# FYTalon/pienerf

Measured on AMD Instinct MI355X. Metric: sim+render steps/s @800x800 chair, higher is better.
Workload: dtype f32 render / f64 sim

## Files before the change

### include/pienerf_hip.h

```cpp
#ifndef PIENERF_HIP_H
#define PIENERF_HIP_H
#include <stdint.h>
#ifdef __cplusplus
extern "C" {
#endif

#define PN_OK 0
#define PN_ERR_ARG 1
#define PN_ERR_HIP 2
#define PN_ERR_CAPACITY 3

const char* pn_version(void);

int pn_stream_create_cu_mask(uint32_t total_cu, uint32_t first_cu, uint32_t n_cu, int invert, void** stream_out);
int pn_stream_destroy(void* stream);
int pn_march_set_tail_rounds(int rounds);
int pn_march_set_skip_dda(int on);
int pn_device_cu_count(void);
const char* pn_last_error(void);


int pn_sph_from_ray(const float* rays_o, const float* rays_d, float radius, uint32_t N, float* coords, void* stream);
int pn_near_far_from_aabb(const float* rays_o, const float* rays_d, const float* aabb, uint32_t N, float min_near, float* nears, float* fars,
                          void* stream);
// ... 148 lines not shown


typedef struct pn_copier pn_copier;
int pn_copier_create(pn_copier** out);
void pn_copier_destroy(pn_copier* c);
int pn_copier_submit(pn_copier* c, void* dst_host, const void* src_dev, uint64_t bytes, void* after_event, uint64_t* ticket);
int pn_copier_wait(pn_copier* c, uint64_t ticket);


int pn_mark_untrained_grid(const float* poses, uint32_t B, float fx, float fy, float cx, float cy, uint32_t cascade, uint32_t H, float bound,
                           float* density_grid, int* n_unseen, void* stream);
int pn_density_cells_full(uint32_t cascade, uint32_t H, float bound, const float* noise, float* xyzs, void* stream);
int pn_density_cells_partial(uint32_t cas, uint32_t H, float bound, uint32_t N, const int* rand_coords, const float* rand_pick, const float* noise,
                             const float* density_grid_cas, float* tmp_grid_cas, int* scratch, int* indices, float* xyzs, void* stream);
uint64_t pn_density_partial_scratch_ints(uint32_t H);
int pn_density_scatter(uint32_t n, const int* indices, const float* sigmas, float* tmp_grid_cas, void* stream);
int pn_density_grid_update(uint32_t n, float* density_grid, const float* tmp_grid, float decay, float density_thresh, uint8_t* bitfield,
                           double* partial, float* mean_thresh, void* stream);

int pn_frame_march_counters(pn_frame* f, int enable, uint64_t* counters_host, void* stream);
int pn_frame_fused_clocks(pn_frame* f, uint64_t* clocks_host, int* first_trip_out, int reset, void* stream);
int pn_frame_trip_records(pn_frame* f, int* records_host, int* tail_counts_host, int max_trips, void* stream);
int pn_frame_trip_times(pn_frame* f, float* march_ms_host, float* network_ms_host, int max_trips, int* n_trips_out, void* stream);


int pn_sim_update_F(int n_IP, const int* topo, const double* dof, const double* Nx, const double* dNx, const double* ddNx, float* pos, float* F,
                    float* dF, void* stream);

int pn_sim_calc_elastic(int n_IP, const int* topo, const double* dNx, const double* dof, double* RF, double* VF, double* FF, int mcadams_sweeps,
                        void* stream);

int pn_sim_collect_rhs(int n_k, double dx, const int* csr_bg, const int* csr_cnt, const int* csr_buf, const double* mu, const double* lam,
                       const double* dNx, const double* RF, const double* VF, double* rhs, void* stream);

int pn_sim_matvec3(int n, const double* A, const double* X, double* Y, void* stream);

int pn_sim_stepforward(int n_k, int n_IP, int iters, double dt, double dx, const int* topo, const int* csr_bg, const int* csr_cnt,
                       const int* csr_buf, const double* mu, const double* lam, const double* dNx, const double* dNx_csr, const int* csr_pos,
                       const double* Ainv,
                       const double* Mmat, const double* dof_rest, const double* rhs_rest, const double* rhs_gravity, const double* dof_f,
                       double* dof, double* dof_vel, double* work, int prepared, int mcadams_sweeps, void* stream);
uint64_t pn_sim_work_doubles(int n_k, int n_IP);
int pn_sim_cells_chunk_ips(void);
uint64_t pn_sim_cells_work_doubles(int n_k, int n_chunks);
int pn_sim_cells_prepare(int n_k, int n_chunks, double* work, void* stream);
int pn_sim_stepforward_cells(int n_k, int n_chunks, int iters, double dt, double dx, const int* chunk_tab, const double* dNx_cell, const double* mu_cell,
// ... 49 lines not shown
```

### pienerf_amd/_lib.py

```python
import ctypes as C
import os

_HERE = os.path.dirname(os.path.abspath(__file__))
LIB_PATH = os.environ.get("PN_LIB_PATH") or os.path.join(_HERE, "lib", "libpienerf_hip.so")

P = C.c_void_p
u32, i32, f32, f64, u64 = C.c_uint32, C.c_int, C.c_float, C.c_double, C.c_uint64


class RenderOpts(C.Structure):
    _fields_ = [("max_iter_num", i32), ("hash_grid_size", f32), ("num_seek_IP", i32), ("IP_dx", f32), ("cut", i32), ("cut_bounds", f32 * 6),
                ("bound", f32), ("min_near", f32), ("dt_gamma", f32), ("max_steps", u32), ("T_thresh", f32), ("cascade", u32), ("grid_size", u32),
                ("density_scale", f32), ("bg_color", f32), ("fp16", i32), ("reuse_tables", i32), ("ray_batch", i32), ("throughput", i32), ("throughput_trips", i32), ("ray_tile_w", i32),
                ("fused_from", i32), ("fused_whole", i32), ("fused_fold", i32), ("fused_grid", i32)]


SIGNATURES = {
    "pn_version": (C.c_char_p, []),
    "pn_last_error": (C.c_char_p, []),
    "pn_stream_create_cu_mask": (i32, [u32, u32, u32, i32, C.POINTER(C.c_void_p)]),
    "pn_stream_destroy": (i32, [P]),
    "pn_device_cu_count": (i32, []),
    "pn_march_set_tail_rounds": (i32, [i32]),
    "pn_march_set_skip_dda": (i32, [i32]),
# ... 44 lines not shown
    "pn_nerf_color_half": (i32, [P, P, P, P, u32, P, P]),
    "pn_render_hier": (i32, [P, P, P, u32, C.POINTER(f32), f32, i32, i32, f32, f32, P, P, P, P, i32, P]),
    "pn_hier_max_samples": (i32, []),
    "pn_frame_create": (i32, [C.POINTER(P), u32, u32, u32]),
    "pn_frame_destroy": (None, [P]),
    "pn_render_deformed": (i32, [P, P, C.POINTER(RenderOpts), P, P, u32, P, P, P, P, i32, P, P, P, P, P, P, P]),
    "pn_render_deformed_async": (i32, [P, P, C.POINTER(RenderOpts), P, P, u32, P, P, P, P, i32, P, P, P, P, P, i32, P]),
    "pn_render_status": (i32, [P, P, i32, P]),
    "pn_frame_reset_unfinished": (i32, [P, P]),
    "pn_render_continue": (i32, [P, P, C.POINTER(RenderOpts), P, P, u32, P, P, P, P, P, P, i32, i32, P]),
    "pn_render_static": (i32, [P, P, C.POINTER(RenderOpts), P, P, u32, P, P, P, P, P, P, P, i32, P]),
    "pn_mark_untrained_grid": (i32, [P, u32, f32, f32, f32, f32, u32, u32, f32, P, P, P]),
    "pn_density_cells_full": (i32, [u32, u32, f32, P, P, P]),
    "pn_density_cells_partial": (i32, [u32, u32, f32, u32, P, P, P, P, P, P, P, P, P]),
    "pn_density_partial_scratch_ints": (u64, [u32]),
    "pn_density_scatter": (i32, [u32, P, P, P, P]),
    "pn_density_grid_update": (i32, [u32, P, P, f32, f32, P, P, P, P]),
    "pn_frame_march_counters": (i32, [P, i32, P, P]),
    "pn_frame_trip_times": (i32, [P, P, P, i32, P, P]),
    "pn_frame_fused_clocks": (i32, [P, P, P, i32, P]),
    "pn_net_form": (i32, [P]),
    "pn_net_form_epoch": (i32, [P]),
    "pn_frame_trip_records": (i32, [P, P, P, i32, P]),
    "pn_sim_update_F": (i32, [i32, P, P, P, P, P, P, P, P, P]),
    "pn_sim_calc_elastic": (i32, [i32, P, P, P, P, P, P, i32, P]),
    "pn_sim_collect_rhs": (i32, [i32, f64, P, P, P, P, P, P, P, P, P, P]),
    "pn_sim_matvec3": (i32, [i32, P, P, P, P]),
    "pn_sim_stepforward": (i32, [i32, i32, i32, f64, f64, P, P, P, P, P, P, P, P, P, P, P, P, P, P, P, P, P, P, i32, i32, P]),
    "pn_sim_prepare": (i32, [i32, i32, P, P, P, P]),
    "pn_sim_cells_chunk_ips": (i32, []),
    "pn_sim_cells_work_doubles": (u64, [i32, i32]),
    "pn_sim_cells_prepare": (i32, [i32, i32, P, P]),
    "pn_sim_stepforward_cells": (i32, [i32, i32, i32, f64, f64, P, P, P, P, P, P, P, P, P, P, P, P, P, P, P, i32, P]),
    "pn_sim_work_doubles": (u64, [i32, i32]),
    "pn_sim_coop_bytes": (u64, [i32, i32, i32]),
    "pn_sim_coop_prepare": (i32, [i32, i32, i32, P, P, P, C.POINTER(i32), P]),
    "pn_sim_coop_status": (i32, [P, C.POINTER(i32)]),
    "pn_sim_coop_clocks": (i32, [P, C.POINTER(u64)]),
    "pn_sim_stepforward_coop": (i32, [i32, i32, i32, f64, f64, P, P, P, P, P, P, P, P, P, P, P, P, P, P, P, P, i32, C.POINTER(i32), P]),
    "pn_sim_update_force": (i32, [i32, i32, P, f64, P, P, P, P, P]),
    "pn_sim_drag_bytes": (u64, []),
    "pn_sim_drag_work_doubles": (u64, []),
    "pn_sim_drag_force": (i32, [i32, i32, P, P, f64, P, P, P, P, P]),
    "pn_sim_drag_set": (i32, [P, i32, i32, i32, f64, P, P]),
    "pn_sim_drag_unproject": (i32, [P, i32, i32, f64, f64, P, P, P, i32, P, P, P]),
    "pn_mc_work_bytes": (u64, [i32, i32, i32]),
# ... 49 lines not shown
```

### pienerf_amd/csrc/pn_render_ops.hip

```cpp
#include <float.h>

#include "pn_render_records.h"
#include "pn_cell_hash.h"
#include "pn_side_tables.h"
#include "pn_march_kernels.h"
#include "pn_composite.h"
#include "pn_compact.h"
#include "pn_frame_kernels.h"

thread_local char pn_err_buf[512] = {0};

extern "C" int pn_pnts_in_grids(int n_vtx, int n_grid, const float* pnts, const float* bbmin, float hgs, const int* resolution, int* pig_cnt,
                                int* pig_bgn, int* pig_idx, int* err_flag, void* stream) {
    PN_REQUIRE(n_vtx > 0 && n_grid > 0 && pnts && bbmin && resolution && pig_cnt && pig_bgn && pig_idx);
    int* cursor = nullptr;
    hipStream_t st = (hipStream_t)stream;
    PN_HIP_CHECK(hipMallocAsync((void**)&cursor, sizeof(int) * (size_t)n_grid, st));
    int rc = pig_build(n_vtx, n_grid, nullptr, pnts, bbmin, hgs, resolution, pig_cnt, pig_bgn, pig_idx, cursor, err_flag, st);
    PN_HIP_CHECK(hipFreeAsync(cursor, st));
    return rc;
}

extern "C" int pn_march_set_skip_dda(int on) {
    PN_REQUIRE(on >= -1 && on <= 1);
// ... 83 lines not shown
    return PN_OK;
}


extern "C" int pn_frame_create(pn_frame** out, uint32_t max_rays, uint32_t max_vtx, uint32_t max_grid_cells) {
    PN_REQUIRE(out && max_rays > 0 && max_vtx > 0 && max_grid_cells > 0);
    pn_frame* f = new pn_frame();
    memset(f, 0, sizeof(*f));
    f->max_rays = max_rays; f->max_vtx = max_vtx; f->max_cells = max_grid_cells;
    const size_t N = max_rays;
#define PN_ALLOC(ptr, bytes) PN_HIP_CHECK(hipMalloc((void**)&(ptr), (bytes)))
    PN_ALLOC(f->nears, N * 4); PN_ALLOC(f->fars, N * 4); PN_ALLOC(f->rays_t, N * 4);
    {
        int dev_id = 0, cus = 0;
        PN_HIP_CHECK(hipGetDevice(&dev_id));
        PN_HIP_CHECK(hipDeviceGetAttribute(&cus, hipDeviceAttributeMultiprocessorCount, dev_id));
        f->fused_blocks = (uint32_t)std::min(std::max(cus, 1), 1024);
    }
    f->blist_cap = (uint32_t)(N / 8 + 64 + (size_t)(f->fused_blocks + 1) * 64);
    const size_t NS = N + (size_t)f->fused_blocks * PN_FUSED_WAVES * 64 + f->blist_cap;
    PN_ALLOC(f->xyzs, NS * 12); PN_ALLOC(f->dirs, NS * 12); PN_ALLOC(f->deltas, NS * 8); PN_ALLOC(f->sigmas, NS * 4); PN_ALLOC(f->rgbs, NS * 12);
    PN_ALLOC(f->fused_ctl, (size_t)PN_FUSED_CTL_INTS * 4);
    PN_HIP_CHECK(hipMemset(f->fused_ctl, 0, (size_t)PN_FUSED_CTL_INTS * 4));
    PN_ALLOC(f->fused_clocks, 16 * sizeof(unsigned long long));
    PN_HIP_CHECK(hipMemset(f->fused_clocks, 0, 16 * sizeof(unsigned long long)));
    f->fused_first = -1;
    PN_ALLOC(f->t_resume, N * 4);
    PN_ALLOC(f->blist, (size_t)f->blist_cap * 8);
    PN_ALLOC(f->strag, (size_t)f->blist_cap * 16);
    PN_ALLOC(f->acc_image, N * 12);
    PN_ALLOC(f->alive_a, N * 4); PN_ALLOC(f->alive_b, N * 4); PN_ALLOC(f->list, N * 4); PN_ALLOC(f->chunk_counts, (N / 256 + 4) * 4);
    PN_ALLOC(f->pig_cnt, (size_t)max_grid_cells * 4); PN_ALLOC(f->pig_bgn, (size_t)max_grid_cells * 4);
    PN_ALLOC(f->pig_cursor, (size_t)max_grid_cells * 4); PN_ALLOC(f->pig_idx, (size_t)max_vtx * 4);
    PN_ALLOC(f->side.nb_rng, ((size_t)max_grid_cells + 1) * sizeof(int2));
    f->side.nb_capacity = 27 * (int)max_vtx;
    PN_ALLOC(f->side.nb, (size_t)f->side.nb_capacity * sizeof(float4)); PN_ALLOC(f->side.rec, (size_t)max_vtx * PN_REC_FLOATS * 4);
    f->seg_cap = seg_cap_for(max_rays);
    PN_ALLOC(f->tail, (size_t)PN_SEGS * f->seg_cap * sizeof(TailEntry)); PN_ALLOC(f->tail_counts, sizeof(int) * (PN_MAX_TRIPS + 2));
    PN_ALLOC(f->list_seg, (size_t)PN_SEGS * f->seg_cap * 4); PN_ALLOC(f->active_seg, (size_t)PN_SEGS * f->seg_cap * 4);
    PN_ALLOC(f->seg_counters, (size_t)6 * PN_SEGS * PN_SEG_STRIDE * 4);
    PN_ALLOC(f->cell_bits, 2 * (((size_t)max_grid_cells + 31) / 32) * 4);
    PN_ALLOC(f->fars_eff, N * 4);
    PN_ALLOC(f->grid_regions, (size_t)PN_GRID_REGION_WORDS * 4);
    PN_ALLOC(f->trips, sizeof(PnTrip) * (PN_MAX_TRIPS + 2)); PN_ALLOC(f->dev, sizeof(PnFrameDev)); PN_ALLOC(f->cut_bounds, 6 * 4);
    f->max_groups = pn_div_up(max_rays, PN_MIN_RAY_BATCH) + 1;
    PN_ALLOC(f->groups, sizeof(PnGroup) * 2 * f->max_groups); PN_ALLOC(f->group_cnt, sizeof(int) * f->max_groups);
#undef PN_ALLOC
    PN_HIP_CHECK(hipMalloc((void**)&f->march_counters, 16 * sizeof(unsigned long long)));
// ... 466 lines not shown
    hipStream_t st = (hipStream_t)stream;
    if (counters_host) {
        PN_HIP_CHECK(hipMemcpyAsync(counters_host, f->march_counters, 4 * sizeof(unsigned long long), hipMemcpyDeviceToHost, st));
#if PN_DBG_PHASES || PN_DBG_STATS
        {
            unsigned long long ph[16];
            PN_HIP_CHECK(hipMemcpy(ph, f->march_counters, sizeof(ph), hipMemcpyDeviceToHost));
            fprintf(stderr, "phases:");
            for (int i = 4; i < 16; i++) fprintf(stderr, " %llu", ph[i]);
            fprintf(stderr, "\n");
        }
#endif
        PN_HIP_CHECK(hipStreamSynchronize(st));
    }
    if ((enable & 1) && !(f->march_counters_on & 1)) PN_HIP_CHECK(hipMemsetAsync(f->march_counters, 0, 16 * sizeof(unsigned long long), st));
    f->march_counters_on = enable & 7;
    return PN_OK;
}

extern "C" int pn_frame_fused_clocks(pn_frame* f, uint64_t* clocks_host, int* first_trip_out, int reset, void* stream) {
    PN_REQUIRE(f);
    hipStream_t st = (hipStream_t)stream;
    if (clocks_host) {
        PN_HIP_CHECK(hipMemcpyAsync(clocks_host, f->fused_clocks, 16 * sizeof(unsigned long long), hipMemcpyDeviceToHost, st));
        PN_HIP_CHECK(hipStreamSynchronize(st));
        clocks_host[15] = f->fused_first >= 0 ? (uint64_t)f->fused_mode : 0u;
    }
    if (first_trip_out) *first_trip_out = f->fused_first;
    if (reset) PN_HIP_CHECK(hipMemsetAsync(f->fused_clocks, 0, 16 * sizeof(unsigned long long), st));
    return PN_OK;
}

extern "C" int pn_frame_trip_times(pn_frame* f, float* march_ms_host, float* network_ms_host, int max_trips, int* n_trips_out, void* stream) {
    PN_REQUIRE(f && march_ms_host && network_ms_host && n_trips_out && max_trips >= 0);
    PN_HIP_CHECK(hipStreamSynchronize((hipStream_t)stream));
    const int n = f->timed_trips < max_trips ? f->timed_trips : max_trips;
    if (f->stamped) {
        static unsigned long long host[PN_TIMED_TRIPS * 3];
        PN_HIP_CHECK(hipMemcpy(host, f->stamps, sizeof(unsigned long long) * (size_t)n * 3, hipMemcpyDeviceToHost));
        for (int t = 0; t < n; t++) {
            march_ms_host[t] = (float)((double)(host[t * 3 + 1] - host[t * 3]) * 1e-5);
            network_ms_host[t] = (float)((double)(host[t * 3 + 2] - host[t * 3 + 1]) * 1e-5);
        }
    } else {
        for (int t = 0; t < n; t++) {
            PN_HIP_CHECK(hipEventElapsedTime(march_ms_host + t, f->ev[t][0], f->ev[t][1]));
            PN_HIP_CHECK(hipEventElapsedTime(network_ms_host + t, f->ev[t][1], f->ev[t][2]));
        }
    }
    *n_trips_out = n;
    return PN_OK;
}

extern "C" int pn_frame_trip_records(pn_frame* f, int* records_host, int* tail_counts_host, int max_trips, void* stream) {
    PN_REQUIRE(f && records_host && tail_counts_host && max_trips >= 0);
    PN_HIP_CHECK(hipStreamSynchronize((hipStream_t)stream));
    const int n = max_trips < PN_MAX_TRIPS ? max_trips : PN_MAX_TRIPS;
    std::vector<PnTrip> rec((size_t)n);
    PN_HIP_CHECK(hipMemcpy(rec.data(), f->trips, sizeof(PnTrip) * (size_t)n, hipMemcpyDeviceToHost));
    for (int i = 0; i < n; i++) {
        int* r = records_host + 5 * i;
        r[0] = rec[i].n_alive; r[1] = rec[i].n_step; r[2] = rec[i].step_base; r[3] = rec[i].n_samples; r[4] = rec[i].dense ? rec[i].n_emitted : -1;
    }
    PN_HIP_CHECK(hipMemcpy(tail_counts_host, f->tail_counts, sizeof(int) * (size_t)n, hipMemcpyDeviceToHost));
    return PN_OK;
}


extern "C" int pn_frame_reset_unfinished(pn_frame* f, void* stream) {
    PN_REQUIRE(f);
    k_reset_unfinished<<<1, 1, 0, (hipStream_t)stream>>>(f->dev);
    PN_LAUNCH_CHECK();
    return PN_OK;
}

extern "C" int pn_render_status(pn_frame* f, int64_t* stats_host, int synchronize, void* stream) {
    PN_REQUIRE(f && stats_host);
    if (synchronize) PN_HIP_CHECK(hipStreamSynchronize((hipStream_t)stream));
    frame_stats(f, stats_host);
    return PN_OK;
}
```

### pienerf_amd/csrc/pn_trips_fused.h

```cpp
#pragma once
#define PN_TU_FP_CONTRACT_OFF 1
#include <cstddef>

#include "pn_net_tile.h"

#define PN_FUSED_MAX_TRIPS 128
#if PN_DBG_PHASES
#define PN_FUSED_PK , pk_dummy_
#else
#define PN_FUSED_PK
#endif
#ifndef PN_FUSED_WROUNDS
#define PN_FUSED_WROUNDS 1
#endif
#ifndef PN_FUSED_WAVES
#define PN_FUSED_WAVES 12
#endif
#ifndef PN_FUSED_LDS_OUT
#define PN_FUSED_LDS_OUT 1
#endif
#ifndef PN_FUSED_LDS_XYZ
#define PN_FUSED_LDS_XYZ 1
#endif
#define PN_FUSED_STAGE 512
#define PN_FUSED_CTL_HIST 0
#define PN_FUSED_CTL_DONE (PN_FUSED_CTL_HIST + 3 * PN_FUSED_MAX_TRIPS)
#define PN_FUSED_CTL_INTS (PN_FUSED_CTL_DONE + 32)

struct FusedArgs {
    const PnFusedLevel* lv;
    const float* emb;
    const uint32_t* emb_h;
    uint32_t emb_bytes;
    const uint4* wimg_g;
    float net_bound, net_inv2b, density_scale;
    const float* x_scales;
    PnTrip* trips;
    uint32_t N_rays, max_steps;
    float T_thresh;
    const int* alive;
    float *rays_t, *weights_sum, *depth, *image;
    float *xyzs, *dirs, *deltas, *sigmas, *rgbs;
    int* ctl;
    PnFrameDev* dev;
    int* tail_diag;
    unsigned long long* clocks;
    const int* active;
    const int* active_counts;
    int active_seg_cap;
    const float* t_resume;
// ... 95 lines not shown
#define PN_FUSED_ACHUNK 64
#endif

template <int K, bool MULTI, int NF, int MODE>
__global__ void __launch_bounds__(PN_FUSED_WAVES * 64, (PN_FUSED_WAVES + 3) / 4) k_trips_fused(pnm::MarchParams a, pnm2::March2Tables tb, FusedArgs fa) {
    extern __shared__ __attribute__((aligned(16))) uint4 fused_lds[];
    constexpr bool HALF = NF == 1, XF = NF == 2;
    constexpr int IMG16 = (HALF ? PN_NET_HALF_BYTES : (XF ? PN_NET_X_BYTES : PN_NET_SPLIT_BYTES)) / 16;
    constexpr int MAXT = PN_FUSED_MAX_TRIPS;
    constexpr int AC = PN_FUSED_ACHUNK;
    static_assert(AC == 64 || AC == 32, "rays per first-trip chunk");
    constexpr bool WHOLE = MODE == 1;
    constexpr bool FOLD = MODE == 2;
    constexpr bool QUEUED = MODE != 0;
    uint4* wimg = fused_lds;
    float4* stage_all = reinterpret_cast<float4*>(fused_lds + IMG16 + 32);
    int* hist = reinterpret_cast<int*>(stage_all + PN_FUSED_WAVES * PN_FUSED_STAGE);
    constexpr bool LXYZ = PN_FUSED_LDS_XYZ != 0 && PN_FUSED_LDS_OUT != 0 && NF != 0;
    float* xyz_all = reinterpret_cast<float*>(hist + 3 * MAXT);
    __shared__ int s_last, s_cursor;
    __shared__ int s_bres, s_bready, s_bhead, s_sres, s_sready, s_shead, s_pending, s_a1done;
    __shared__ int s_pend[PN_FUSED_MAXCHUNKS];
    __shared__ int s_pref[PN_SEGS + 1];

#if PN_DBG_PHASES
    pnm3::PhaseClock pk_dummy_;
#endif
    const PnTrip* tr = fa.trips;
    const int lane = threadIdx.x & 63, wv = threadIdx.x >> 6;
    if (PN_FUSED_FRESH_ARGS && blockIdx.x == 0 && threadIdx.x == 0) {
        const FusedArgs& fk = fused_args_fresh(fa);
        const pnm::MarchParams& ak = fused_karg_fresh<pnm::MarchParams, 0>(a);
        const pnm2::March2Tables& tk = fused_karg_fresh<pnm2::March2Tables, 1>(tb);
        if (fk.trips != fa.trips || fk.rays_t != fa.rays_t || fk.N_rays != fa.N_rays || fk.image_out != fa.image_out || fk.seg_back != fa.seg_back || ak.rays_o != a.rays_o ||
            ak.grid != a.grid || ak.hgs != a.hgs || tk.nb != tb.nb || tk.rec != tb.rec) atomicOr(&fa.dev->err, 32);
    }
    const float x_scale = XF ? fa.x_scales[0] : 1.0f, x_rscale = XF ? fa.x_scales[1] : 1.0f;
    int A = 0, sb0 = 0, n_active = 0;
    if (QUEUED) {
        if (threadIdx.x < 64) {
            const int cnt = seg_count(WHOLE ? fa.active_counts : fa.samp_counts, lane);
            int inc = cnt;
#pragma unroll
            for (int o = 1; o < 64; o <<= 1) {
                const int u = __shfl_up(inc, o);
                if (lane >= o) inc += u;
            }
            s_pref[lane + 1] = inc;
            if (lane == 0) s_pref[0] = 0;
        }
        __syncthreads();
        n_active = s_pref[PN_SEGS];
        const long long chunks = ((long long)n_active + AC - 1) / AC;
        const bool ok = tr->n_alive == (int)fa.N_rays && tr->n_step == 1 && tr->step_base == 0 && (long long)n_active * 8 <= (long long)fa.N_rays &&
                        (chunks + (long long)gridDim.x) * AC <= (long long)fa.blist_cap &&
                        (WHOLE ? (chunks + (long long)gridDim.x - 1) / (long long)gridDim.x <= PN_FUSED_MAXCHUNKS : true);
        if (!ok) return;
        sb0 = 1;
    } else {
        A = tr->n_alive; sb0 = tr->step_base;
        if (!(A > 0 && tr->n_step == 8 && tr->dense != 0)) return;
    }

    for (int i = threadIdx.x; i < IMG16; i += PN_FUSED_WAVES * 64) wimg[i] = fa.wimg_g[i];
    if (threadIdx.x < 16 * sizeof(PnFusedLevel) / 16) wimg[IMG16 + threadIdx.x] = reinterpret_cast<const uint4*>(fa.lv)[threadIdx.x];
    for (int i = threadIdx.x; i < 3 * MAXT; i += PN_FUSED_WAVES * 64) hist[i] = 0;
    if (threadIdx.x == 0) { s_cursor = 0; s_bres = s_bready = s_bhead = s_sres = s_sready = s_shead = s_a1done = 0; }
    if (QUEUED) {
        const int n_items0 = WHOLE ? (n_active + AC - 1) / AC : (n_active + 31) / 32;
        const int mine0 = (int)blockIdx.x < n_items0 ? (n_items0 - (int)blockIdx.x + (int)gridDim.x - 1) / (int)gridDim.x : 0;
        if (threadIdx.x == 0) s_pending = mine0;
        if (WHOLE)
            for (int i = threadIdx.x; i < PN_FUSED_MAXCHUNKS; i += PN_FUSED_WAVES * 64) s_pend[i] = 64;
    }
    __syncthreads();

    const int sub = lane & 7, gbase = lane & ~7, grp = lane >> 3;
    const uint32_t wave_g = blockIdx.x * PN_FUSED_WAVES + wv;
    const uint32_t slotw = (FOLD ? fa.N_rays : 0u) + wave_g * 64u, slot0 = slotw + (uint32_t)grp * 8u;
    float4* stage = stage_all + wv * PN_FUSED_STAGE;
    const uint4* __restrict__ wl = wimg + lane;
    const int half = lane >> 5, s32 = lane & 31;
    const PnFusedLevel* lds_lv = reinterpret_cast<const PnFusedLevel*>(wimg + IMG16) + 8 * half;
    __amdgpu_buffer_rsrc_t emb_rsrc = __builtin_amdgcn_make_buffer_rsrc(const_cast<uint32_t*>(fa.emb_h), 0, (int)fa.emb_bytes, 0x00020000);
    float* const X = LXYZ ? xyz_all + wv * 192 + grp * 24 : fa.xyzs + (size_t)slot0 * 3;
    float* const Dd = LXYZ ? nullptr : fa.dirs + (size_t)slot0 * 3;
    float* const dl = fa.deltas + (size_t)slot0 * 2;

    const bool clk = fa.clocks != nullptr;
    unsigned long long c_acc[10] = {0, 0, 0, 0, 0, 0, 0, 0, 0, 0}, c_t = 0, rounds = 0;
// ... 65 lines not shown
    int share = 0;
    const int* my_list = nullptr;
    int my_chunks = 0;
    int *a_index = nullptr, *blist = nullptr;
    int4* strag = nullptr;
    uint32_t a_base = 0;
    bool go_on = true;
    auto lds_ld = [](int* p_) __attribute__((always_inline)) { return __hip_atomic_load(p_, __ATOMIC_RELAXED, __HIP_MEMORY_SCOPE_WORKGROUP); };
    auto lds_st = [](int* p_, int v) __attribute__((always_inline)) { __hip_atomic_store(p_, v, __ATOMIC_RELAXED, __HIP_MEMORY_SCOPE_WORKGROUP); };
    auto q_claim = [&](int* head, int* ready, int want, int& take) __attribute__((always_inline)) {
        int base = 0;
        take = 0;
        for (;;) {
            const int h = lds_ld(head), r = lds_ld(ready);
            const int t_ = min(want, r - h);
            if (t_ <= 0) break;
            if (atomicCAS(head, h, h + t_) == h) { base = h; take = t_; break; }
        }
        return base;
    };
    auto q_publish = [&](int* ready, int base, int n) __attribute__((always_inline)) {
        while (lds_ld(ready) != base) __builtin_amdgcn_s_sleep(1);
        lds_st(ready, base + n);
    };
    auto chunk_finish = [&](int ci) __attribute__((always_inline)) {
#pragma unroll 1
        for (int tile = 0; tile < AC / 32; tile++) {
            const int pos = ci * AC + tile * 32 + s32;
            const uint32_t slot = a_base + (uint32_t)pos;
            const bool has = fa.deltas[(size_t)slot * 2] != 0.0f;
            const unsigned long long em = __ballot(has && half == 0);
            if (!em) continue;
            if (lane == 0) {
                atomicAdd(&hist[MAXT], (int)__popcll(em));
                if (a.stats) atomicAdd(a.stats + 3, (unsigned long long)__popcll(em));
            }
            network_tile(slot);
            wave_sync_mem();
            tick(7);
            bool on = false;
            int idx = -1;
            if (has && half == 0) {
                idx = a_index[pos];
                on = composite_one(idx, slot, 1u, fa.T_thresh, fa.rays_t, fa.sigmas, fa.rgbs, fa.deltas, fa.weights_sum, fa.depth, fa.image) && go_on;
                if (!on && fa.finalize) finalize_ray(fa, idx);
            }
// ... 102 lines not shown
                if (s2.step == 0u && lane < 8) {
                    if (lane < 2) fa.deltas[sl * 2 + lane] = 0.0f;
                    else if (lane < 5) fa.xyzs[sl * 3 + (lane - 2)] = 0.0f;
                    else fa.dirs[sl * 3 + (lane - 5)] = 0.0f;
                }
                wave_sync_mem();
                tick(6);
                if (chunk_arrive(se.x / AC, 1)) fin_chunk = se.x / AC;
            }
            if (fin_chunk >= 0) chunk_finish(fin_chunk);
            if (ci < my_chunks || got) continue;
            int gone = 0;
            if (lane == 0) gone = (lds_ld(&s_a1done) >= my_chunks && lds_ld(&s_shead) >= lds_ld(&s_sready)) ? 1 : 0;
            if (__builtin_amdgcn_readfirstlane(gone)) break;
            __builtin_amdgcn_s_sleep(16);
            tick(9);
        }
    }

    bool pool_empty = false;
    int index = -1;
    int j = 0;

    for (;;) {
        if (QUEUED || !pool_empty) {
            const unsigned long long em = __ballot(index < 0 && sub == 0);
            const int need = (int)__popcll(em);
            if (need > 0) {
                const int my_rank = (int)__popcll(em & ((1ull << gbase) - 1ull));
                int base = 0, take = need;
                if (QUEUED) {
                    if (lane == 0) base = q_claim(&s_bhead, &s_bready, need, take);
                    take = __builtin_amdgcn_readfirstlane(take);
                } else {
                    if (lane == 0) base = atomicAdd(&s_cursor, need);
                }
                base = __builtin_amdgcn_readfirstlane(base);
                if (!QUEUED) pool_empty = base + need >= share;
                const int p = base + my_rank;
                const int gpos = QUEUED ? p : ((p >> 3) * (int)gridDim.x + (int)blockIdx.x) * 8 + (p & 7);
                if (index < 0 && (QUEUED ? my_rank < take : (p < share && gpos < A))) {
                    index = QUEUED ? my_list[gpos] : fa.alive[gpos];
                    j = QUEUED ? 1 : 0;
                    pnm3::RayConsts cn;
                    pnm3::ray_consts(a, index, cn);
                    r_ox = cn.ox; r_oy = cn.oy; r_oz = cn.oz; r_dx = cn.dx; r_dy = cn.dy; r_dz = cn.dz; r_rdx = cn.rdx; r_rdy = cn.rdy; r_rdz = cn.rdz; r_far = cn.far;
                    r_t = a.rays_t[index];
                }
            }
        }
        bool fold_round = false, f_has = false;
        uint32_t f_slot = 0u;
        if (!__any(index >= 0)) {
            if (!QUEUED) break;
            if (FOLD) {
                int ti = my_chunks;
                if (lane == 0 && lds_ld(&s_cursor) < my_chunks) ti = atomicAdd(&s_cursor, 1);
                ti = __builtin_amdgcn_readfirstlane(ti);
                if (ti < my_chunks) {
                    fold_round = true;
                    const int e = ((int)blockIdx.x + ti * (int)gridDim.x) * 32 + s32;
                    f_has = e < n_active;
                    if (f_has) {
                        int lo = 0, hi = PN_SEGS;
                        while (hi - lo > 1) {
                            const int mid = (lo + hi) >> 1;
                            if (s_pref[mid] <= e) lo = mid; else hi = mid;
                        }
                        f_slot = (uint32_t)fa.list_seg[(size_t)lo * fa.list_seg_cap + (e - s_pref[lo])];
                    }
                    f_slot = f_has ? f_slot : (uint32_t)__builtin_amdgcn_readlane((int)f_slot, (int)__builtin_ctzll(__ballot(f_has)));
                }
            }
            if (!fold_round) {
                int fin = 0;
                if (lane == 0) fin = (lds_ld(&s_pending) == 0 && lds_ld(&s_bhead) >= lds_ld(&s_bready)) ? 1 : 0;
                if (__builtin_amdgcn_readfirstlane(fin)) break;
                __builtin_amdgcn_s_sleep(32);
                tick(9);
                continue;
            }
        }
        unsigned long long net_mask = 0ull;
        bool have_ray = false;
        if (fold_round) {
            net_mask = __ballot(f_has && half == 0);
            if (lane == 0) atomicAdd(&hist[MAXT], (int)__popcll(net_mask));
            tick(0);
        } else {
        rounds++;
        tick(0);
        have_ray = index >= 0;
        if (have_ray && sub == 0) atomicAdd(&hist[j], 1);
        const pnm::MarchParams& am = fused_karg_fresh<pnm::MarchParams, 0>(a);
        const pnm2::March2Tables& tbm = fused_karg_fresh<pnm2::March2Tables, 1>(tb);
        pnm3::RayConsts c;
        pnm3::frame_consts(am, c);
        c.ox = r_ox; c.oy = r_oy; c.oz = r_oz; c.dx = r_dx; c.dy = r_dy; c.dz = r_dz; c.rdx = r_rdx; c.rdy = r_rdy; c.rdz = r_rdz; c.far = r_far;
        pnm3::RayState st{0.f, 0.f, 0u};
        bool have = false;
        if (have_ray) {
            float t = r_t;
            t += pnm::clampf(t * am.dt_gamma, c.dt_min, c.dt_max) * 0.0f;
            st.last_t = t;
            st.t = t;
            have = t < c.far;
        }
        const bool done = pnm3::march_window<K, MULTI, 8, PN_FUSED_STAGE, 1>(am, tbm, c, 8u, sub, gbase, lane, stage, X, Dd, dl, st, PN_FUSED_WROUNDS, have PN_FUSED_PK);
        const bool deferred = have && !done;
        tick(1);
        unsigned long long dm = __ballot(deferred && sub == 0);
        if (deferred && sub == 0) atomicAdd(&hist[2 * MAXT + j], 1);
        while (dm) {
            const int L = (int)__builtin_ctzll(dm);
            dm &= dm - 1ull;
            pnm3::RayConsts c2;
            pnm3::frame_consts(am, c2);
            c2.ox = readlane_f(c.ox, L); c2.oy = readlane_f(c.oy, L); c2.oz = readlane_f(c.oz, L);
            c2.dx = readlane_f(c.dx, L); c2.dy = readlane_f(c.dy, L); c2.dz = readlane_f(c.dz, L);
            c2.rdx = readlane_f(c.rdx, L); c2.rdy = readlane_f(c.rdy, L); c2.rdz = readlane_f(c.rdz, L);
            c2.far = readlane_f(c.far, L);
            pnm3::RayState s2{readlane_f(st.t, L), readlane_f(st.last_t, L), (uint32_t)__builtin_amdgcn_readlane((int)st.step, L)};
            const size_t sl = (size_t)slotw + (size_t)(L >> 3) * 8;
            pnm3::march_window<K, MULTI, 64, PN_FUSED_STAGE, 1>(am, tbm, c2, 8u, lane, 0, lane, stage, LXYZ ? xyz_all + wv * 192 + (L >> 3) * 24 : fa.xyzs + sl * 3,
                                                                LXYZ ? nullptr : fa.dirs + sl * 3, fa.deltas + sl * 2, s2, 0x7fffffff, true PN_FUSED_PK);
            if (gbase == L) st.step = s2.step;
        }
        const uint32_t emitted = have_ray ? st.step : 0u;
        if (have_ray && sub == 0 && emitted) {
            atomicAdd(&hist[MAXT + j], (int)emitted);
            if (a.stats) atomicAdd(a.stats + 3, (unsigned long long)emitted);
        }
        if (have_ray && (uint32_t)sub >= emitted) {
            dl[2 * sub] = 0.0f; dl[2 * sub + 1] = 0.0f;
            X[3 * sub] = X[3 * sub + 1] = X[3 * sub + 2] = 0.0f;
// ... 6 lines not shown
        network64(net_mask, !fold_round, f_slot);
        wave_sync_mem();
        tick(fold_round ? 7 : 3);
        if (fold_round) {
            bool on = false;
            int idx = -1;
            if (f_has && half == 0) {
                idx = fa.alive[f_slot];
                on = composite_one(idx, f_slot, 1u, fa.T_thresh, fa.rays_t, fa.sigmas, fa.rgbs, fa.deltas, fa.weights_sum, fa.depth, fa.image) && go_on;
                if (!on && fa.finalize) finalize_ray(fa, idx);
            }
            const unsigned long long om = __ballot(on);
            wave_sync_mem();
            if (om) {
                int base = 0;
                if (lane == 0) base = atomicAdd(&s_bres, (int)__popcll(om));
                base = __builtin_amdgcn_readfirstlane(base);
                if (on) blist[base + (int)__popcll(om & ((1ull << lane) - 1ull))] = idx;
                wave_sync_mem();
                if (lane == 0) q_publish(&s_bready, base, (int)__popcll(om));
            }
            if (lane == 0) atomicSub(&s_pending, 1);
            tick(8);
            continue;
        }
        int alive = 0;
        const FusedArgs& fc = fused_args_fresh(fa);
        if (have_ray && sub == 0)
            alive = composite_slots8<PN_FUSED_LDS_OUT != 0>(index, slot0, fc.T_thresh, r_t, fc.rays_t, fc.sigmas, fc.rgbs, fc.deltas, fc.weights_sum, fc.depth, fc.image,
                                                            stage + grp * 8) ? 1 : 0;
        alive = __shfl(alive, gbase);
        r_t = __shfl(r_t, gbase);
        if (have_ray) {
            if (alive && (uint32_t)(sb0 + 8 * (j + (QUEUED ? 0 : 1))) < fa.max_steps && j + 1 < MAXT) j++;
            else {
                if (QUEUED && fc.finalize && sub == 0) finalize_ray(fc, index);
                index = -1;
            }
        }
        tick(4);
    }
    if (clk && lane == 0) {
        for (int k = 0; k < 5; k++) atomicAdd(fa.clocks + k, c_acc[k]);
        atomicAdd(fa.clocks + 5, rounds);
        atomicAdd(fa.clocks + 6, 1ull);
        atomicAdd(fa.clocks + 7, __builtin_amdgcn_s_memrealtime() - rt0);
        atomicMax(fa.clocks + 8, rounds);
        atomicMax(fa.clocks + 9, __builtin_amdgcn_s_memrealtime() - rt0);
        if (QUEUED)
            for (int k = 5; k < 10; k++) atomicAdd(fa.clocks + 5 + k, c_acc[k]);
    }

    __syncthreads();
    for (int i = threadIdx.x; i < 3 * MAXT; i += PN_FUSED_WAVES * 64) {
        const int v = hist[i];
        if (v) atomicAdd(fa.ctl + PN_FUSED_CTL_HIST + i, v);
    }
    asm volatile("s_waitcnt vmcnt(0)" ::: "memory");
    __syncthreads();
    if (threadIdx.x == 0) {
        const int old = atomicAdd(fa.ctl + PN_FUSED_CTL_DONE, 1);
        s_last = (old == (int)gridDim.x - 1) ? 1 : 0;
    }
    __syncthreads();
    if (!s_last || threadIdx.x >= 64) return;
    int m = 0;
    long long n_samples_total = 0;
    for (int j0 = 0; j0 < MAXT; j0 += 64) {
        const int jj = j0 + lane;
        int* hp = fa.ctl + PN_FUSED_CTL_HIST + jj;
        int al = __hip_atomic_load(hp, __ATOMIC_RELAXED, __HIP_MEMORY_SCOPE_AGENT);
// ... 84 lines not shown
```

### pienerf_amd/nerf/renderer.py

```python
import ctypes as C
import math

import torch
import torch.nn as nn

from .. import raymarching
from .._lib import RenderOpts, check, lib, ptr, require_gpu, stream_ptr
from .utils import get_pnts_in_grids


def _flat_rays(rays_o, rays_d):
    return rays_o.to(torch.float32).contiguous().view(-1, 3), rays_d.to(torch.float32).contiguous().view(-1, 3)


def sample_pdf(bins, weights, n_samples, det=False):
    if weights.shape[-1] < 1:
        raise RuntimeError("sample_pdf: no bin weights (the hierarchical sampler needs num_steps >= 3: weights[:, 1:-1] is empty)")
    weights = weights + 1e-5
    pdf = weights / torch.sum(weights, -1, keepdim=True)
    cdf = torch.cumsum(pdf, -1)
    cdf = torch.cat([torch.zeros_like(cdf[..., :1]), cdf], -1)
    if det:
        u = torch.linspace(0. + 0.5 / n_samples, 1. - 0.5 / n_samples, steps=n_samples).to(weights.device)
        u = u.expand(list(cdf.shape[:-1]) + [n_samples])
# ... 176 lines not shown
        if static:
            o = self._static_opts(dt_gamma, 1 if bg_color is None else bg_color, max_steps, T_thresh)
        else:
            o = self._deformed_opts(dt_gamma, 1 if bg_color is None else bg_color, max_steps, T_thresh, kwargs, n_rays=N)
        image, depth, ws = out["image"].view(-1, 3), out["depth"].view(-1), out["weights_sum"].view(-1)
        depth_0 = out["depth_0"].view(-1) if "depth_0" in out else torch.empty_like(depth)
        assert image.is_contiguous() and image.shape[0] == N
        stats = (C.c_int64 * 5)() if int(n_trips) == 0 else None
        check(lib().pn_render_continue(self._frames[slot][0], self._net_handle(half=bool(o.fp16)), C.byref(o), ptr(rays_o), ptr(rays_d), N,
                                       ptr(self.density_bitfield), ptr(image), ptr(depth), ptr(depth_0), ptr(ws), stats, int(n_trips), int(bool(static)),
                                       stream_ptr()), "render_continue")
        if self.bg_radius > 0:
            self.blend_background(rays_o, rays_d, ws, image)
        if stats is not None:
            self._set_stats(stats)
        return out

    def _set_stats(self, stats):
        self.last_stats = dict(trips=int(stats[0]), samples=int(stats[1]), err=int(stats[2]), alive_at_exit=int(stats[3]), unfinished=int(stats[4]))
        if stats[2]:
            raise RuntimeError(f"render_deformed: device error flags {int(stats[2])} (1: sample cell outside the spatial hash, "
                               "2: IP outside it, 4: spatial-hash capacity exceeded, 8: candidate-list capacity exceeded, "
                               "16: the fused composite/compaction gave up waiting for an earlier chunk, 32: the fused launch found its kernarg segment laid "
                               "out otherwise than csrc/pn_trips_fused.h: fused_karg_fresh assumes)")

    def march_counters(self, enable, read=False, slot=0):
        out = (C.c_uint64 * 4)() if read else None
        check(lib().pn_frame_march_counters(self._frames[slot][0], int(enable), out, stream_ptr()), "march_counters")
        return None if out is None else dict(iterations=int(out[0]), candidates=int(out[1]), warps=int(out[2]), samples=int(out[3]))

    def fused_clocks(self, slot=0, reset=False):
        out, first = (C.c_uint64 * 16)(), C.c_int(-1)
        check(lib().pn_frame_fused_clocks(self._frames[slot][0], out, C.byref(first), int(bool(reset)), stream_ptr()), "fused_clocks")
        return dict(refill=int(out[0]), march=int(out[1]), windows=int(out[2]), network=int(out[3]), composite=int(out[4]), wave_rounds=int(out[5]),
                    waves=int(out[6]), lifetime_ticks=int(out[7]), max_rounds=int(out[8]), max_lifetime_ticks=int(out[9]), first_trip=int(first.value),
                    a_march=int(out[10]), a_windows=int(out[11]), a_network=int(out[12]), a_composite=int(out[13]), a_barrier=int(out[14]),
                    mode=int(out[15]))

    def trip_records(self, slot=0, max_trips=16):
        rec, tail = (C.c_int * (5 * max_trips))(), (C.c_int * max_trips)()
        check(lib().pn_frame_trip_records(self._frames[slot][0], rec, tail, max_trips, stream_ptr()), "trip_records")
        return [tuple(rec[5 * i:5 * i + 5]) + (tail[i],) for i in range(max_trips) if rec[5 * i] > 0]

    def trip_times(self, slot=0):
        a, b, n = (C.c_float * 64)(), (C.c_float * 64)(), C.c_int(0)
        check(lib().pn_frame_trip_times(self._frames[slot][0], a, b, 64, C.byref(n), stream_ptr()), "trip_times")
        return [float(a[i]) for i in range(n.value)], [float(b[i]) for i in range(n.value)]

    def render_status(self, synchronize=True, slot=0):
        stats = (C.c_int64 * 5)()
        check(lib().pn_render_status(self._frames[slot][0], stats, int(bool(synchronize)), stream_ptr()), "render_status")
        self._set_stats(stats)
        return self.last_stats

    def reset_extra_state(self):
        if not self.cuda_ray:
            return
        self.density_grid.zero_()
        self.mean_density = 0
        self.iter_density = 0
# ... 307 lines not shown
```

Baseline: 1484.

## Add per-workgroup straggler ring so idle waves steal deferred rays in fused march

Adds an LDS ring queue per workgroup to the fused march/network kernel. Rays whose march window is deferred get pushed onto it, and idle waves pop up to two of them to process on their behalf. Termination now also waits for the busy count and an empty ring, with an idle cap that raises a new error flag. This aims to reduce load imbalance from straggler rays holding a workgroup's lifetime, at the cost of extra atomics and sync overhead and a risk of livelock. Also adds diagnostic clocks and a rays_t readback function.

```diff
diff --git a/include/pienerf_hip.h b/include/pienerf_hip.h
--- a/include/pienerf_hip.h
+++ b/include/pienerf_hip.h
@@ -194,6 +194,7 @@
 int pn_frame_fused_clocks(pn_frame* f, uint64_t* clocks_host, int* first_trip_out, int reset, void* stream);
 int pn_frame_trip_records(pn_frame* f, int* records_host, int* tail_counts_host, int max_trips, void* stream);
 int pn_frame_trip_times(pn_frame* f, float* march_ms_host, float* network_ms_host, int max_trips, int* n_trips_out, void* stream);
+int pn_frame_rays_t(pn_frame* f, float* rays_t_host, uint32_t n, void* stream);
 
 
 int pn_sim_update_F(int n_IP, const int* topo, const double* dof, const double* Nx, const double* dNx, const double* ddNx, float* pos, float* F,
diff --git a/pienerf_amd/_lib.py b/pienerf_amd/_lib.py
--- a/pienerf_amd/_lib.py
+++ b/pienerf_amd/_lib.py
@@ -90,6 +90,7 @@
     "pn_net_form": (i32, [P]),
     "pn_net_form_epoch": (i32, [P]),
     "pn_frame_trip_records": (i32, [P, P, P, i32, P]),
+    "pn_frame_rays_t": (i32, [P, P, u32, P]),
     "pn_sim_update_F": (i32, [i32, P, P, P, P, P, P, P, P, P]),
     "pn_sim_calc_elastic": (i32, [i32, P, P, P, P, P, P, i32, P]),
     "pn_sim_collect_rhs": (i32, [i32, f64, P, P, P, P, P, P, P, P, P, P]),
diff --git a/pienerf_amd/csrc/pn_render_ops.hip b/pienerf_amd/csrc/pn_render_ops.hip
--- a/pienerf_amd/csrc/pn_render_ops.hip
+++ b/pienerf_amd/csrc/pn_render_ops.hip
@@ -129,8 +129,8 @@
     PN_ALLOC(f->xyzs, NS * 12); PN_ALLOC(f->dirs, NS * 12); PN_ALLOC(f->deltas, NS * 8); PN_ALLOC(f->sigmas, NS * 4); PN_ALLOC(f->rgbs, NS * 12);
     PN_ALLOC(f->fused_ctl, (size_t)PN_FUSED_CTL_INTS * 4);
     PN_HIP_CHECK(hipMemset(f->fused_ctl, 0, (size_t)PN_FUSED_CTL_INTS * 4));
-    PN_ALLOC(f->fused_clocks, 16 * sizeof(unsigned long long));
-    PN_HIP_CHECK(hipMemset(f->fused_clocks, 0, 16 * sizeof(unsigned long long)));
+    PN_ALLOC(f->fused_clocks, PN_FUSED_CLOCK_WORDS * sizeof(unsigned long long));
+    PN_HIP_CHECK(hipMemset(f->fused_clocks, 0, PN_FUSED_CLOCK_WORDS * sizeof(unsigned long long)));
     f->fused_first = -1;
     PN_ALLOC(f->t_resume, N * 4);
     PN_ALLOC(f->blist, (size_t)f->blist_cap * 8);
@@ -643,12 +643,14 @@
     PN_REQUIRE(f);
     hipStream_t st = (hipStream_t)stream;
     if (clocks_host) {
-        PN_HIP_CHECK(hipMemcpyAsync(clocks_host, f->fused_clocks, 16 * sizeof(unsigned long long), hipMemcpyDeviceToHost, st));
+        PN_HIP_CHECK(hipMemcpyAsync(clocks_host, f->fused_clocks, PN_FUSED_CLOCK_WORDS * sizeof(unsigned long long), hipMemcpyDeviceToHost, st));
         PN_HIP_CHECK(hipStreamSynchronize(st));
+        clocks_host[19] = clocks_host[18] >> 32;
+        clocks_host[18] &= 0xFFFFFFFFull;
         clocks_host[15] = f->fused_first >= 0 ? (uint64_t)f->fused_mode : 0u;
     }
     if (first_trip_out) *first_trip_out = f->fused_first;
-    if (reset) PN_HIP_CHECK(hipMemsetAsync(f->fused_clocks, 0, 16 * sizeof(unsigned long long), st));
+    if (reset) PN_HIP_CHECK(hipMemsetAsync(f->fused_clocks, 0, PN_FUSED_CLOCK_WORDS * sizeof(unsigned long long), st));
     return PN_OK;
 }
 
@@ -687,6 +689,12 @@
     return PN_OK;
 }
 
+extern "C" int pn_frame_rays_t(pn_frame* f, float* rays_t_host, uint32_t n, void* stream) {
+    PN_REQUIRE(f && rays_t_host && n <= f->max_rays);
+    PN_HIP_CHECK(hipStreamSynchronize((hipStream_t)stream));
+    PN_HIP_CHECK(hipMemcpy(rays_t_host, f->rays_t, sizeof(float) * (size_t)n, hipMemcpyDeviceToHost));
+    return PN_OK;
+}
 
 extern "C" int pn_frame_reset_unfinished(pn_frame* f, void* stream) {
     PN_REQUIRE(f);
diff --git a/pienerf_amd/csrc/pn_trips_fused.h b/pienerf_amd/csrc/pn_trips_fused.h
--- a/pienerf_amd/csrc/pn_trips_fused.h
+++ b/pienerf_amd/csrc/pn_trips_fused.h
@@ -22,10 +22,16 @@
 #ifndef PN_FUSED_LDS_XYZ
 #define PN_FUSED_LDS_XYZ 1
 #endif
+#ifndef PN_FUSED_QTAKE
+#define PN_FUSED_QTAKE 2
+#endif
+#define PN_FUSED_QCAP 32
+#define PN_FUSED_IDLE_CAP (1 << 20)
 #define PN_FUSED_STAGE 512
 #define PN_FUSED_CTL_HIST 0
 #define PN_FUSED_CTL_DONE (PN_FUSED_CTL_HIST + 3 * PN_FUSED_MAX_TRIPS)
 #define PN_FUSED_CTL_INTS (PN_FUSED_CTL_DONE + 32)
+#define PN_FUSED_CLOCK_WORDS 20
 
 struct FusedArgs {
     const PnFusedLevel* lv;
@@ -167,6 +173,8 @@
     __shared__ int s_bres, s_bready, s_bhead, s_sres, s_sready, s_shead, s_pending, s_a1done;
     __shared__ int s_pend[PN_FUSED_MAXCHUNKS];
     __shared__ int s_pref[PN_SEGS + 1];
+    __shared__ int s_qres, s_qhead, s_busy;
+    __shared__ unsigned long long s_q[PN_FUSED_QCAP];
 
 #if PN_DBG_PHASES
     pnm3::PhaseClock pk_dummy_;
@@ -210,7 +218,8 @@
     for (int i = threadIdx.x; i < IMG16; i += PN_FUSED_WAVES * 64) wimg[i] = fa.wimg_g[i];
     if (threadIdx.x < 16 * sizeof(PnFusedLevel) / 16) wimg[IMG16 + threadIdx.x] = reinterpret_cast<const uint4*>(fa.lv)[threadIdx.x];
     for (int i = threadIdx.x; i < 3 * MAXT; i += PN_FUSED_WAVES * 64) hist[i] = 0;
-    if (threadIdx.x == 0) { s_cursor = 0; s_bres = s_bready = s_bhead = s_sres = s_sready = s_shead = s_a1done = 0; }
+    if (threadIdx.x == 0) { s_cursor = 0; s_bres = s_bready = s_bhead = s_sres = s_sready = s_shead = s_a1done = 0; s_qres = s_qhead = s_busy = 0; }
+    if (threadIdx.x < PN_FUSED_QCAP) s_q[threadIdx.x] = ~0ull;
     if (QUEUED) {
         const int n_items0 = WHOLE ? (n_active + AC - 1) / AC : (n_active + 31) / 32;
         const int mine0 = (int)blockIdx.x < n_items0 ? (n_items0 - (int)blockIdx.x + (int)gridDim.x - 1) / (int)gridDim.x : 0;
@@ -322,6 +331,28 @@
     auto q_publish = [&](int* ready, int base, int n) __attribute__((always_inline)) {
         while (lds_ld(ready) != base) __builtin_amdgcn_s_sleep(1);
         lds_st(ready, base + n);
+    };
+    auto sq_push = [&](int idx, int jj) __attribute__((always_inline)) {
+        for (int tries = 0; tries < 64; tries++) {
+            const int r = lds_ld(&s_qres), h = lds_ld(&s_qhead);
+            if (r - h >= PN_FUSED_QCAP) return false;
+            if (atomicCAS(&s_qres, r, r + 1) == r) {
+                const unsigned long long e = ((unsigned long long)((unsigned)r & 0xFFFFFFu) << 40) | ((unsigned long long)(unsigned)jj << 32) | (unsigned long long)(unsigned)idx;
+                __hip_atomic_store(&s_q[r & (PN_FUSED_QCAP - 1)], e, __ATOMIC_RELEASE, __HIP_MEMORY_SCOPE_WORKGROUP);
+                return true;
+            }
+        }
+        return false;
+    };
+    auto sq_pop = [&]() __attribute__((always_inline)) {
+        for (int tries = 0; tries < 16; tries++) {
+            const int h = lds_ld(&s_qhead), r = lds_ld(&s_qres);
+            if (h >= r) break;
+            const unsigned long long e = __hip_atomic_load(&s_q[h & (PN_FUSED_QCAP - 1)], __ATOMIC_ACQUIRE, __HIP_MEMORY_SCOPE_WORKGROUP);
+            if ((unsigned)(e >> 40) != ((unsigned)h & 0xFFFFFFu)) break;
+            if (atomicCAS(&s_qhead, h, h + 1) == h) return e;
+        }
+        return ~0ull;
     };
     auto chunk_finish = [&](int ci) __attribute__((always_inline)) {
 #pragma unroll 1
@@ -470,7 +501,43 @@
     int index = -1;
     int j = 0;
 
+    bool counted = false;
+    bool pushed_last = false;
+    int idle = 0;
+    unsigned long long n_def_wave = 0, rt_last = rt0;
+    auto load_ray = [&]() __attribute__((always_inline)) {
+        pnm3::RayConsts cn;
+        pnm3::ray_consts(a, index, cn);
+        r_ox = cn.ox; r_oy = cn.oy; r_oz = cn.oz; r_dx = cn.dx; r_dy = cn.dy; r_dz = cn.dz; r_rdx = cn.rdx; r_rdy = cn.rdy; r_rdz = cn.rdz; r_far = cn.far;
+        r_t = a.rays_t[index];
+    };
+
     for (;;) {
+        bool wide = false;
+        if (PN_FUSED_QTAKE > 0) {
+            unsigned long long fm = __ballot(index < 0 && sub == 0);
+            if (fm && !(pushed_last && __any(index >= 0))) {
+                int avail = 0;
+                if (lane == 0) avail = lds_ld(&s_qres) - lds_ld(&s_qhead);
+                if (__builtin_amdgcn_readfirstlane(avail) > 0) {
+                    for (int k = 0; k < PN_FUSED_QTAKE && fm; k++) {
+                        unsigned long long e = ~0ull;
+                        if (lane == 0) e = sq_pop();
+                        const int qi = __builtin_amdgcn_readfirstlane((int)(unsigned)e), qh = __builtin_amdgcn_readfirstlane((int)(unsigned)(e >> 32));
+                        if (qi < 0) break;
+                        const int G = (int)__builtin_ctzll(fm);
+                        fm &= fm - 1ull;
+                        if (gbase == G) {
+                            index = qi;
+                            j = qh & 0xFF;
+                            wide = true;
+                            load_ray();
+                        }
+                    }
+                }
+            }
+            pushed_last = false;
+        }
         if (QUEUED || !pool_empty) {
             const unsigned long long em = __ballot(index < 0 && sub == 0);
             const int need = (int)__popcll(em);
@@ -490,17 +557,18 @@
                 if (index < 0 && (QUEUED ? my_rank < take : (p < share && gpos < A))) {
                     index = QUEUED ? my_list[gpos] : fa.alive[gpos];
                     j = QUEUED ? 1 : 0;
-                    pnm3::RayConsts cn;
-                    pnm3::ray_consts(a, index, cn);
-                    r_ox = cn.ox; r_oy = cn.oy; r_oz = cn.oz; r_dx = cn.dx; r_dy = cn.dy; r_dz = cn.dz; r_rdx = cn.rdx; r_rdy = cn.rdy; r_rdz = cn.rdz; r_far = cn.far;
-                    r_t = a.rays_t[index];
+                    load_ray();
                 }
             }
         }
         bool fold_round = false, f_has = false;
         uint32_t f_slot = 0u;
-        if (!__any(index >= 0)) {
-            if (!QUEUED) break;
+        const bool any_ray = __any(index >= 0);
+        if (any_ray != counted) {
+            if (lane == 0) atomicAdd(&s_busy, any_ray ? 1 : -1);
+            counted = any_ray;
+        }
+        if (!any_ray) {
             if (FOLD) {
                 int ti = my_chunks;
                 if (lane == 0 && lds_ld(&s_cursor) < my_chunks) ti = atomicAdd(&s_cursor, 1);
@@ -522,13 +590,20 @@
             }
             if (!fold_round) {
                 int fin = 0;
-                if (lane == 0) fin = (lds_ld(&s_pending) == 0 && lds_ld(&s_bhead) >= lds_ld(&s_bready)) ? 1 : 0;
-                if (__builtin_amdgcn_readfirstlane(fin)) break;
+                if (lane == 0)
+                    fin = ((QUEUED ? (lds_ld(&s_pending) == 0 && lds_ld(&s_bhead) >= lds_ld(&s_bready)) : true) && lds_ld(&s_busy) == 0 &&
+                           lds_ld(&s_qhead) >= lds_ld(&s_qres)) ? 1 : 0;
+                if (__builtin_amdgcn_readfirstlane(fin) && (QUEUED || pool_empty)) break;
+                if (++idle > PN_FUSED_IDLE_CAP) {
+                    if (lane == 0) atomicOr(&fa.dev->err, 64);
+                    break;
+                }
                 __builtin_amdgcn_s_sleep(32);
                 tick(9);
                 continue;
             }
         }
+        idle = 0;
         unsigned long long net_mask = 0ull;
         bool have_ray = false;
         if (fold_round) {
@@ -539,7 +614,7 @@
         rounds++;
         tick(0);
         have_ray = index >= 0;
-        if (have_ray && sub == 0) atomicAdd(&hist[j], 1);
+        if (have_ray && sub == 0 && !wide) atomicAdd(&hist[j], 1);
         const pnm::MarchParams& am = fused_karg_fresh<pnm::MarchParams, 0>(a);
         const pnm2::March2Tables& tbm = fused_karg_fresh<pnm2::March2Tables, 1>(tb);
         pnm3::RayConsts c;
@@ -554,11 +629,28 @@
             st.t = t;
             have = t < c.far;
         }
-        const bool done = pnm3::march_window<K, MULTI, 8, PN_FUSED_STAGE, 1>(am, tbm, c, 8u, sub, gbase, lane, stage, X, Dd, dl, st, PN_FUSED_WROUNDS, have PN_FUSED_PK);
-        const bool deferred = have && !done;
+        const bool done = pnm3::march_window<K, MULTI, 8, PN_FUSED_STAGE, 1>(am, tbm, c, 8u, sub, gbase, lane, stage, X, Dd, dl, st, PN_FUSED_WROUNDS, have && !wide PN_FUSED_PK);
+        const bool deferred = have && !wide && !done;
         tick(1);
         unsigned long long dm = __ballot(deferred && sub == 0);
         if (deferred && sub == 0) atomicAdd(&hist[2 * MAXT + j], 1);
+        if (clk) n_def_wave += (unsigned long long)__popcll(dm);
+        if (PN_FUSED_QTAKE > 0 && dm) {
+            wave_sync_mem();
+            unsigned long long rest = dm, pm = 0ull;
+            while (rest) {
+                const int L = (int)__builtin_ctzll(rest);
+                rest &= rest - 1ull;
+                const int qi = __builtin_amdgcn_readlane(index, L), qj = __builtin_amdgcn_readlane(j, L);
+                int ok = 0;
+                if (lane == 0) ok = sq_push(qi, qj) ? 1 : 0;
+                if (__builtin_amdgcn_readfirstlane(ok)) pm |= 1ull << L;
+            }
+            if ((pm >> gbase) & 1ull) { index = -1; have_ray = false; }
+            dm &= ~pm;
+            pushed_last = pm != 0ull;
+        }
+        dm |= __ballot(wide && have && sub == 0);
         while (dm) {
             const int L = (int)__builtin_ctzll(dm);
             dm &= dm - 1ull;
@@ -611,6 +703,7 @@
             }
             if (lane == 0) atomicSub(&s_pending, 1);
             tick(8);
+            if (clk) rt_last = __builtin_amdgcn_s_memrealtime();
             continue;
         }
         int alive = 0;
@@ -628,14 +721,19 @@
             }
         }
         tick(4);
+        if (clk) rt_last = __builtin_amdgcn_s_memrealtime();
     }
     if (clk && lane == 0) {
         for (int k = 0; k < 5; k++) atomicAdd(fa.clocks + k, c_acc[k]);
         atomicAdd(fa.clocks + 5, rounds);
         atomicAdd(fa.clocks + 6, 1ull);
-        atomicAdd(fa.clocks + 7, __builtin_amdgcn_s_memrealtime() - rt0);
+        const unsigned long long life = rt_last - rt0;
+        atomicAdd(fa.clocks + 7, life);
         atomicMax(fa.clocks + 8, rounds);
-        atomicMax(fa.clocks + 9, __builtin_amdgcn_s_memrealtime() - rt0);
+        atomicMax(fa.clocks + 9, life);
+        atomicMax(fa.clocks + 16, c_acc[2]);
+        atomicMax(fa.clocks + 17, n_def_wave);
+        atomicMax(fa.clocks + 18, (life << 32) | (c_acc[2] < 0xFFFFFFFFull ? c_acc[2] : 0xFFFFFFFFull));
         if (QUEUED)
             for (int k = 5; k < 10; k++) atomicAdd(fa.clocks + 5 + k, c_acc[k]);
     }
diff --git a/pienerf_amd/nerf/renderer.py b/pienerf_amd/nerf/renderer.py
--- a/pienerf_amd/nerf/renderer.py
+++ b/pienerf_amd/nerf/renderer.py
@@ -222,7 +222,8 @@
             raise RuntimeError(f"render_deformed: device error flags {int(stats[2])} (1: sample cell outside the spatial hash, "
                                "2: IP outside it, 4: spatial-hash capacity exceeded, 8: candidate-list capacity exceeded, "
                                "16: the fused composite/compaction gave up waiting for an earlier chunk, 32: the fused launch found its kernarg segment laid "
-                               "out otherwise than csrc/pn_trips_fused.h: fused_karg_fresh assumes)")
+                               "out otherwise than csrc/pn_trips_fused.h: fused_karg_fresh assumes, 64: a wave of the fused launch gave up waiting for its workgroup's "
+                               "straggler ring to drain)")
 
     def march_counters(self, enable, read=False, slot=0):
         out = (C.c_uint64 * 4)() if read else None
@@ -230,12 +231,18 @@
         return None if out is None else dict(iterations=int(out[0]), candidates=int(out[1]), warps=int(out[2]), samples=int(out[3]))
 
     def fused_clocks(self, slot=0, reset=False):
-        out, first = (C.c_uint64 * 16)(), C.c_int(-1)
+        out, first = (C.c_uint64 * 20)(), C.c_int(-1)
         check(lib().pn_frame_fused_clocks(self._frames[slot][0], out, C.byref(first), int(bool(reset)), stream_ptr()), "fused_clocks")
         return dict(refill=int(out[0]), march=int(out[1]), windows=int(out[2]), network=int(out[3]), composite=int(out[4]), wave_rounds=int(out[5]),
                     waves=int(out[6]), lifetime_ticks=int(out[7]), max_rounds=int(out[8]), max_lifetime_ticks=int(out[9]), first_trip=int(first.value),
                     a_march=int(out[10]), a_windows=int(out[11]), a_network=int(out[12]), a_composite=int(out[13]), a_barrier=int(out[14]),
-                    mode=int(out[15]))
+                    mode=int(out[15]),
+                    max_windows=int(out[16]), max_deferred=int(out[17]), longest_windows=int(out[18]), longest_lifetime_ticks=int(out[19]))
+
+    def frame_rays_t(self, n, slot=0):
+        out = torch.empty(int(n), dtype=torch.float32)
+        check(lib().pn_frame_rays_t(self._frames[slot][0], C.c_void_p(out.data_ptr()), int(n), stream_ptr()), "frame_rays_t")
+        return out
 
     def trip_records(self, slot=0, max_trips=16):
         rec, tail = (C.c_int * (5 * max_trips))(), (C.c_int * max_trips)()
```

Result: no change. 1480 (-0.3%).
